# flawyer/Celebrity-Image-Denoiser

Hardware: AMD Instinct MI355X
Metric: images/sec at batch 256, 128x128x3, fp32 denoise forward (higher is better)
Workload: dtype f32

## Files before the change

celebrity_image_denoiser_amd/_lib.py:

```python
from __future__ import annotations

import ctypes
import os

_HERE = os.path.dirname(os.path.abspath(__file__))
LIB_PATH = os.environ.get("CID_LIB_PATH") or os.path.join(_HERE, "libcid.so")

CID_OK = 0
CID_NUM_PARAMS = 24
CID_NUM_LAUNCHES = 12
CID_ALGO_DIRECT, CID_ALGO_WINOGRAD64, CID_ALGO_WINOGRAD42, CID_ALGO_SPLIT16 = 0, 2, 3, 4
CID_FMT_F32_NCHW, CID_FMT_U8_NHWC = 0, 1
CID_DTYPE_F32, CID_DTYPE_F16 = 0, 1
CID_TAIL_FUSED, CID_TAIL_BANDS, CID_TAIL_TILES = 0, 1, 2
CID_METRIC_PSNR, CID_METRIC_SSIM, CID_METRIC_MS_SSIM = 1, 2, 4
CID_DISC_MOMENTUM_NONE = -1.0
CID_NOISE_GAUSSIAN, CID_NOISE_SALT_PEPPER, CID_NOISE_SPECKLE, CID_NOISE_POISSON, CID_NOISE_UNIFORM = 0, 1, 2, 3, 4
CID_ADAM_MAX_TENSORS = 32
CID_RESAMPLE_BICUBIC = 3
CID_SR_RAW = 1
CID_CG_RAW = 1
CID_LPIPS_UNIT_VIEW = 1
CID_LPIPS_NUM_WEIGHTS = 17

# ... 17 lines not shown
    "cid_set_weight": (_c.c_int, [_c.c_void_p, _c.c_char_p, _c.c_void_p, _c.POINTER(_c.c_int64), _c.c_int]),
    "cid_get_weight": (_c.c_int, [_c.c_void_p, _c.c_char_p, _c.c_void_p, _c.c_size_t]),
    "cid_missing_weights": (_c.c_int, [_c.c_void_p, _c.POINTER(_c.c_int)]),
    "cid_param_key": (_c.c_char_p, [_c.c_int]),
    "cid_packed_weights_bytes": (_c.c_size_t, []),
    "cid_upload_weights": (_c.c_int, [_c.c_void_p, _c.c_void_p, _c.c_void_p]),
    "cid_pack_weights_device": (_c.c_int, [_c.c_void_p, _c.c_void_p, _c.c_void_p, _c.c_void_p]),
    "cid_packed_segment": (_c.c_int, [_c.c_int, _c.POINTER(_c.c_char_p), _c.POINTER(_c.c_size_t), _c.POINTER(_c.c_size_t)]),
    "cid_export_packed": (_c.c_int, [_c.c_void_p, _c.c_void_p, _c.c_size_t]),
    "cid_import_packed": (_c.c_int, [_c.c_void_p, _c.c_void_p, _c.c_size_t]),
    "cid_attach_weights": (_c.c_int, [_c.c_void_p, _c.c_void_p]),
    "cid_out_shape": (_c.c_int, [_c.c_int, _c.c_int, _c.POINTER(_c.c_int), _c.POINTER(_c.c_int)]),
    "cid_workspace_bytes": (_c.c_int, [_c.c_int, _c.c_int, _c.c_int, _c.POINTER(_c.c_size_t)]),
    "cid_forward": (_c.c_int, [_c.c_void_p, _c.c_void_p, _c.c_void_p, _c.c_int, _c.c_int, _c.c_int,
                               _c.c_void_p, _c.c_size_t, _c.c_void_p]),
    "cid_forward_ex": (_c.c_int, [_c.c_void_p, _c.c_void_p, _c.c_int, _c.c_void_p, _c.c_int, _c.c_int, _c.c_int, _c.c_int,
                                  _c.c_void_p, _c.c_size_t, _c.c_void_p]),
    "cid_forward_padded": (_c.c_int, [_c.c_void_p, _c.c_void_p, _c.c_int, _c.c_void_p, _c.c_int, _c.c_int, _c.c_int, _c.c_int,
                                      _c.c_int, _c.c_int, _c.c_int, _c.c_int, _c.c_void_p, _c.c_size_t, _c.c_void_p]),
    "cid_view_u8": (_c.c_int, [_c.c_void_p, _c.c_void_p, _c.c_int, _c.c_int, _c.c_int, _c.c_void_p]),
    "cid_forward_timed": (_c.c_int, [_c.c_void_p, _c.c_void_p, _c.c_void_p, _c.c_int, _c.c_int, _c.c_int,
                                     _c.c_void_p, _c.c_size_t, _c.c_void_p, _c.POINTER(_c.c_float)]),
    "cid_timing_begin": (_c.c_int, [_c.c_void_p, _c.c_int]),
    "cid_timing_end": (_c.c_int, [_c.c_void_p, _c.c_void_p, _c.POINTER(_c.c_float), _c.POINTER(_c.c_int)]),
    "cid_launch_name": (_c.c_char_p, [_c.c_int]),
    "cid_launch_kernel": (_c.c_char_p, [_c.c_void_p, _c.c_int]),
    "cid_set_conv_algo": (_c.c_int, [_c.c_void_p, _c.c_int]),
    "cid_get_conv_algo": (_c.c_int, [_c.c_void_p, _c.POINTER(_c.c_int)]),
    "cid_set_tail_algo": (_c.c_int, [_c.c_void_p, _c.c_int]),
    "cid_get_tail_algo": (_c.c_int, [_c.c_void_p, _c.POINTER(_c.c_int)]),
    "cid_debug_poison_lds": (_c.c_int, [_c.c_void_p]),
    "cid_debug_winograd_workgroups_per_cu": (_c.c_int, [_c.c_int]),
    "cid_debug_half_workgroups_per_cu": (_c.c_int, [_c.c_int]),
    "cid_debug_winograd_column_block_per_xcd": (_c.c_int, [_c.c_int]),
    "cid_set_compute_dtype": (_c.c_int, [_c.c_void_p, _c.c_int]),
    "cid_get_compute_dtype": (_c.c_int, [_c.c_void_p, _c.POINTER(_c.c_int)]),
    "cid_launch_work_ex": (_c.c_int, [_c.c_void_p, _c.c_int, _c.c_int, _c.c_int, _c.c_int, _c.POINTER(_c.c_double), _c.POINTER(_c.c_double)]),
    "cid_stage_view": (_c.c_int, [_c.c_char_p, _c.c_int, _c.c_int, _c.c_int, _c.POINTER(_c.c_size_t), _c.POINTER(_c.c_int),
                                  _c.POINTER(_c.c_int), _c.POINTER(_c.c_int), _c.POINTER(_c.c_int), _c.POINTER(_c.c_int)]),
    "cid_comm_available": (_c.c_int, []),
    "cid_comm_unique_id": (_c.c_int, [_c.c_void_p]),
    "cid_comm_init_rank": (_c.c_int, [_c.POINTER(_c.c_void_p), _c.c_int, _c.c_void_p, _c.c_int]),
    "cid_comm_destroy": (_c.c_int, [_c.c_void_p]),
    "cid_comm_count": (_c.c_int, [_c.c_void_p, _c.POINTER(_c.c_int)]),
    "cid_broadcast_weights": (_c.c_int, [_c.c_void_p, _c.c_void_p, _c.c_int, _c.c_int, _c.c_void_p]),
    "cid_launch_work": (_c.c_int, [_c.c_int, _c.c_int, _c.c_int, _c.c_int, _c.POINTER(_c.c_double), _c.POINTER(_c.c_double)]),
    "cid_quality_workspace_bytes": (_c.c_int, [_c.c_int, _c.c_int, _c.c_int, _c.c_int, _c.POINTER(_c.c_size_t)]),
    "cid_quality": (_c.c_int, [_c.c_void_p, _c.c_int, _c.c_void_p, _c.c_int, _c.c_int, _c.c_int, _c.c_int, _c.c_int,
                               _c.c_void_p, _c.c_void_p, _c.c_size_t, _c.c_void_p]),
    "cid_add_noise": (_c.c_int, [_c.c_void_p, _c.c_void_p, _c.c_int, _c.c_int, _c.c_int, _c.c_int, _c.POINTER(_c.c_double), _c.c_int,
                                 _c.c_uint64, _c.c_uint64, _c.c_void_p]),
    "cid_disc_create": (_c.c_int, [_c.POINTER(_c.c_void_p)]),
    "cid_disc_destroy": (None, [_c.c_void_p]),
    "cid_disc_last_error": (_c.c_char_p, [_c.c_void_p]),
    "cid_disc_set_weight": (_c.c_int, [_c.c_void_p, _c.c_char_p, _c.c_void_p, _c.POINTER(_c.c_int64), _c.c_int]),
    "cid_disc_packed_weights_bytes": (_c.c_size_t, []),
    "cid_disc_upload_weights": (_c.c_int, [_c.c_void_p, _c.c_void_p, _c.c_void_p]),
    "cid_disc_workspace_bytes": (_c.c_int, [_c.c_int, _c.c_int, _c.c_int, _c.c_int, _c.POINTER(_c.c_size_t)]),
    "cid_disc_forward": (_c.c_int, [_c.c_void_p, _c.c_void_p, _c.c_int, _c.c_void_p, _c.c_int, _c.c_int, _c.c_int, _c.c_void_p,
                                    _c.c_int, _c.c_void_p, _c.c_size_t, _c.c_void_p]),
    "cid_disc_saved_bytes": (_c.c_int, [_c.c_int, _c.c_int, _c.c_int, _c.c_int, _c.POINTER(_c.c_size_t)]),
    "cid_disc_forward_saved": (_c.c_int, [_c.c_void_p, _c.c_void_p, _c.c_int, _c.c_void_p, _c.c_int, _c.c_int, _c.c_int, _c.c_void_p,
                                          _c.c_int, _c.c_void_p, _c.c_size_t, _c.c_void_p]),
    "cid_disc_backward_workspace_bytes": (_c.c_int, [_c.c_int, _c.c_int, _c.c_int, _c.c_int, _c.POINTER(_c.c_size_t)]),
    "cid_disc_backward": (_c.c_int, [_c.c_void_p, _c.c_void_p, _c.c_int, _c.c_void_p, _c.c_int, _c.c_int, _c.c_int, _c.c_void_p,
                                     _c.c_int, _c.c_void_p, _c.c_size_t, _c.c_void_p, _c.c_void_p, _c.c_size_t, _c.c_void_p]),
# ... 141 lines not shown
```

celebrity_image_denoiser_amd/csrc/cid_api.hip:

```cpp
#include "../../include/cid.h"
#include "conv_kernels.h"
#include "wino64_kernels.h"
#include "wino42_kernels.h"
#include "conv_kernels_f16.h"
#include "quality_kernels.h"
#include "noise_kernels.h"
#include "disc_kernels.h"
#include "disc_bwd_kernels.h"
#include "gen_bwd_kernels.h"
#include "gen_pack_kernels.h"
#include "optim_kernels.h"
#include "resize_kernels.h"
#include "esrgan_kernels.h"
#include "srgan_kernels.h"
#include "cgan_kernels.h"
#include "lpips_kernels.h"

#include <dlfcn.h>

#include <algorithm>
#include <atomic>
#include <cmath>

#include <cstdio>
// ... 187 lines not shown

enum Buf { T0, CAT1, P1, T1, CAT2, P2, T2, BT, T3, D2, T4, NBUF };
struct Plan { size_t off[NBUF]; size_t total_bytes; };
Plan make_plan(const Dims& d) {
    const size_t s0 = (size_t)d.N * d.H * d.W, s1 = (size_t)d.N * d.H1 * d.W1, s2 = (size_t)d.N * d.H2 * d.W2;
    const size_t su2 = (size_t)d.N * d.Hu2 * d.Wu2, su1 = (size_t)d.N * d.Hu1 * d.Wu1;
    const size_t sz[NBUF] = {s0 * 64, su1 * 128, s1 * 64, s1 * 128, su2 * 256, s2 * 128, s2 * 256, s2 * 256, su2 * 128, su2 * 128, su1 * 64};
    Plan p; size_t o = 0;
    for (int b = 0; b < NBUF; ++b) { p.off[b] = o; o = align_up(o + sz[b], 64); }
    p.total_bytes = o * sizeof(float);
    return p;
}

}

struct cid_handle_s {
    std::vector<float> staging;
    bool have[NL][2];
    const float* dev_blob = nullptr;
    std::string err;
    int dtype = CID_DTYPE_F32;
    int tail_algo = CID_TAIL_FUSED;
    int algo = CID_ALGO_WINOGRAD42;
    std::vector<hipEvent_t> tev;
    int tev_forwards = 0, tev_used = 0;
    cid_handle_s() : staging(kBlob.total, 0.f) {
        std::memset(have, 0, sizeof(have));
        stage_segments(staging.data(), kTables, nullptr);
    }
};

namespace {

struct Config { int dtype, algo, tail; };
Config config_of(cid_handle_t h) {
    return h ? Config{h->dtype, h->algo, h->tail_algo} : Config{CID_DTYPE_F32, CID_ALGO_DIRECT, CID_TAIL_BANDS};
}

enum class Kern {
    HEAD, HEAD_H16,
    GEMM,
    CONVT_S32,
    WINO64, WINO42,
    SPLIT, SPLIT_PAIR,
    H16, CONVT_T16,
    Z_WINO64, Z_WINO42, Z_SPLIT, Z_H16,
    TAIL_BANDS, TAIL_TILES, TAIL_H,
    TAIL_Z, TAIL_ZH,
};

Kern select_kernel(const Config& c, int i) {
    const LayerDef& L = kLayers[i];
    const bool f16 = c.dtype == CID_DTYPE_F16;
    const bool fused = c.tail == CID_TAIL_FUSED && (f16 || c.algo != CID_ALGO_DIRECT);
    switch (L.kind) {
        case HEAD: return f16 ? Kern::HEAD_H16 : Kern::HEAD;
        case TAIL:
            if (fused) return f16 ? Kern::TAIL_ZH : Kern::TAIL_Z;
            return f16 ? Kern::TAIL_H : c.tail == CID_TAIL_BANDS ? Kern::TAIL_BANDS : Kern::TAIL_TILES;
        case CONVT:
            if (f16) return Kern::CONVT_T16;
            if (c.algo == CID_ALGO_SPLIT16) return Kern::SPLIT_PAIR;
            return L.cin == 128 ? Kern::CONVT_S32 : Kern::GEMM;
        case CONV: break;
    }
    const bool z = fused && i == 10;
    if (f16) return z ? Kern::Z_H16 : Kern::H16;
    switch (c.algo) {
        case CID_ALGO_WINOGRAD64: return z ? Kern::Z_WINO64 : Kern::WINO64;
        case CID_ALGO_WINOGRAD42: return z ? Kern::Z_WINO42 : Kern::WINO42;
        case CID_ALGO_SPLIT16: return z ? Kern::Z_SPLIT : L.cout >= 128 ? Kern::SPLIT_PAIR : Kern::SPLIT;
        default: return Kern::GEMM;
    }
}

std::string kernel_name(const Config& c, int i) {
    const LayerDef& L = kLayers[i];
    const std::string dims = std::to_string(L.cin) + ", " + std::to_string(L.cout);
    const std::string mode = dims + ", " + std::to_string(mode_of(L)) + ",", pool = dims + (L.pool ? ", true," : ", false,");
    switch (select_kernel(c, i)) {
        case Kern::HEAD: return "k_conv_head";
        case Kern::HEAD_H16: return "k_conv_head_h16";
        case Kern::GEMM: return "k_gemm_conv<" + dims + ", " + std::to_string(mode_of(L));
        case Kern::CONVT_S32: return "k_convt_s32<" + dims + ">";
        case Kern::WINO64: case Kern::Z_WINO64: return "k_wino64_conv<" + pool;
        case Kern::WINO42: case Kern::Z_WINO42: return "k_wino42_conv<" + pool;
        case Kern::SPLIT: case Kern::SPLIT_PAIR: return "k_conv3x3_h16<" + mode + " false, false, true,";
        case Kern::H16: return "k_conv3x3_h16<" + mode + (i == 10 ? " false," : "");
        case Kern::CONVT_T16: return "k_convt_t16<" + dims + ">";
        case Kern::Z_SPLIT: return "k_conv3x3_h16<" + mode + " true, false, true,";
        case Kern::Z_H16: return "k_conv3x3_h16<" + mode + " true,";
        case Kern::TAIL_BANDS: case Kern::TAIL_TILES: return "k_conv_tail";
        case Kern::TAIL_H: return "k_conv_tail_h<";
        case Kern::TAIL_Z: return c.algo == CID_ALGO_SPLIT16 ? "k_conv_tail_z<" : "k_conv_tail";
        case Kern::TAIL_ZH: return "k_conv_tail_zh<";
    }
    return "";
}
struct KernelNames {
    std::string s[2][CID_ALGO_SPLIT16 + 1][3][NL];
    KernelNames() {
        for (int dt = 0; dt < 2; ++dt)
            for (int algo = 0; algo <= CID_ALGO_SPLIT16; ++algo)
                for (int tail = 0; tail < 3; ++tail)
                    for (int i = 0; i < NL; ++i) s[dt][algo][tail][i] = kernel_name(Config{dt, algo, tail}, i);
    }
};
const KernelNames kKernelNames;

int fail(cid_handle_t h, int code, const std::string& msg) {
    if (h) h->err = msg;
    return code;
}

bool find_key(const char* key, int& layer, int& is_bias) {
    if (!key) return false;
    const std::string k(key);
    for (int l = 0; l < NL; ++l) {
        const std::string n(kLayers[l].name);
        if (k == n + ".weight") { layer = l; is_bias = 0; return true; }
        if (k == n + ".bias") { layer = l; is_bias = 1; return true; }
    }
    return false;
}

inline int cdiv(int a, int b) { return (a + b - 1) / b; }

template <typename A>
void set_tiles(A& a, int N, int Hc, int Wc, int tw, int th) {
    a.tiles_x = cdiv(Wc, tw); a.tiles_y = cdiv(Hc, th); a.tiles_total = N * a.tiles_x * a.tiles_y;
    a.rcp_x = tile_rcp(a.tiles_x); a.rcp_xy = tile_rcp(a.tiles_x * a.tiles_y);
    if constexpr (std::is_same_v<A, HeadArgs> || std::is_same_v<A, TailArgs>) tile_groups(a);
    else a.tiles_per_xcd = cdiv(a.tiles_total, 8);
}

struct LayerIO {
    const float* in; int Hin, Win, in_ps;
    float* out; int out_ps, out_coff;
// ... 27 lines not shown
    if (hipGetDevice(&dev) != hipSuccess || dev < 0 || dev >= MAXDEV) return 256;
    int n = cache[dev].load(std::memory_order_relaxed);
    if (n > 0) return n;
    if (hipDeviceGetAttribute(&n, hipDeviceAttributeMultiprocessorCount, dev) != hipSuccess || n < 1) n = 256;
    cache[dev].store(n, std::memory_order_relaxed);
    return n;
}
int wino42_grid(WinoArgs& a, int nb) {
    const int per_cu = g_wino42_wg_per_cu;
    const int cus = device_cus();
    const int items = 8 * a.tiles_per_xcd * nb;
    const int walkers = per_cu * cus / 8;
    a.walk = 0;
    if (per_cu <= 0 || walkers < 1 || items <= 8 * walkers || a.tiles_per_xcd < walkers) return items;
    a.walk = walkers;
    if ((nb == 2 || nb == 4) && (g_wino42_xnb & nb)) {
        a.tiles_per_xcd = cdiv(a.tiles_total, 8 / nb);
        a.walk = -walkers;
    }
    return 8 * walkers;
}

template <int CIN, int COUT, int MODE>
hipError_t launch_gemm(const Ctx& x, int layer, const LayerIO& io) {
    GemmConvArgs a;
    set_layer_io(a, x.N, io);
    a.w = x.blob + kBlob.w_off[layer]; a.bias = x.blob + kBlob.b_off[layer];
    set_tiles(a, x.N, io.Hc, io.Wc, TILE_W, TILE_H);
    constexpr int NB = (MODE == 2 ? 4 * COUT : COUT) / NTILE;
    hipLaunchKernelGGL((k_gemm_conv<CIN, COUT, MODE>), dim3(8 * a.tiles_per_xcd * NB), dim3(THREADS), 0, x.s, a);
    return hipGetLastError();
}

template <int CIN, int COUT>
hipError_t launch_convt_s32(const Ctx& x, int layer, const LayerIO& io) {
    using CG = ConvTGeom32<CIN, COUT>;
    GemmConvArgs a;
    set_layer_io(a, x.N, io);
    a.w = x.blob + kBlob.w_off[layer]; a.bias = x.blob + kBlob.b_off[layer];
    a.tiles_x = (io.Hin * io.Win + CG::TP - 1) / CG::TP; a.tiles_y = 1; a.tiles_total = x.N * a.tiles_x; a.tiles_per_xcd = 0;
    a.rcp_x = tile_rcp(a.tiles_x); a.rcp_xy = tile_rcp(io.Win);
    const int wgs = device_cus() * 2;
    hipLaunchKernelGGL((k_convt_s32<CIN, COUT>), dim3(a.tiles_total < wgs ? a.tiles_total : wgs), dim3(THREADS), 0, x.s, a);
    return hipGetLastError();
}

template <bool ZOUT>
WinoArgs wino_args(const Ctx& x, int layer, const LayerIO& io, size_t u_off) {
    WinoArgs a;
    set_layer_io(a, x.N, io);
    a.u = x.blob + u_off; a.bias = x.blob + kBlob.b_off[layer];
    a.zw = ZOUT ? x.blob + kBlob.w_off[11] : nullptr; a.zout = ZOUT ? io.out : nullptr;
    if (ZOUT) a.out = nullptr;
    a.walk = 0;
    return a;
}

template <int CIN, int COUT, bool POOL, bool ZOUT>
hipError_t launch_wino64(const Ctx& x, int layer, const LayerIO& io) {
    WinoArgs a = wino_args<ZOUT>(x, layer, io, kBlob.u_off[layer]);
    const bool wide = io.Wc > 32;
    a.slot_tab = reinterpret_cast<const unsigned*>(x.blob + kBlob.tab_off[wide ? 0 : 1]);
    set_tiles(a, x.N, io.Hc, io.Wc, wide ? 64 : 32, wide ? 2 : 4);
    const dim3 grid(8 * a.tiles_per_xcd * (COUT / WN2));
    if (wide) hipLaunchKernelGGL((k_wino64_conv<CIN, COUT, POOL, 32, ZOUT>), grid, dim3(THREADS), 0, x.s, a);
    else hipLaunchKernelGGL((k_wino64_conv<CIN, COUT, POOL, 16, ZOUT>), grid, dim3(THREADS), 0, x.s, a);
    return hipGetLastError();
}

template <int CIN, int COUT, bool POOL, bool ZOUT>
hipError_t launch_wino42(const Ctx& x, int layer, const LayerIO& io) {
    WinoArgs a = wino_args<ZOUT>(x, layer, io, kBlob.u42_off[layer]);
    const bool wide = io.Wc > 16;
    a.slot_tab = reinterpret_cast<const unsigned*>(x.blob + kBlob.tab42_off[wide ? 0 : 1]);
    set_tiles(a, x.N, io.Hc, io.Wc, wide ? 32 : 16, wide ? 4 : 8);
    const dim3 grid(wino42_grid(a, COUT / WN2));
// ... 18 lines not shown

template <int CIN, int COUT, int MODE, bool ZOUT>
hipError_t launch_gemm_h(const Ctx& x, int layer, const LayerIO& io) {
    GemmConvArgsH a;
    set_layer_io(a, x.N, io);
    a.w = reinterpret_cast<const _Float16*>(x.blob + kBlob.h_off[layer]); a.bias = x.blob + kBlob.b_off[layer];
    if (ZOUT) a.pool = const_cast<_Float16*>(reinterpret_cast<const _Float16*>(x.blob + kBlob.hz_off));
    set_tiles(a, x.N, io.Hc, io.Wc, TILE_W, TILE_H);
    constexpr int NB = (MODE == 2 ? 4 * COUT : COUT) / NTILE;
    a.walk = 0;
    if constexpr (MODE == 2 && !ZOUT) {
        using CG = ConvTGeom<CIN, COUT>;
        a.tiles_x = (io.Hin * io.Win + CG::TP - 1) / CG::TP; a.tiles_total = x.N * a.tiles_x;
        a.rcp_x = tile_rcp(a.tiles_x); a.rcp_xy = tile_rcp(io.Win);
        const int wgs = device_cus() * 2 / CG::CB;
        hipLaunchKernelGGL((k_convt_t16<CIN, COUT>), dim3(a.tiles_total < wgs ? a.tiles_total : wgs), dim3(64 * CG::NW), 0, x.s, a);
    } else if constexpr (MODE != 2) {
        if (io.in_ps != CIN) return hipErrorInvalidValue;
        int grid = 8 * a.tiles_per_xcd * NB;
        const int walkers = g_half_wg_per_cu * device_cus() / 8;
        if (CIN <= 128 && g_half_wg_per_cu > 0 && walkers >= 1 && grid > 8 * walkers && a.tiles_per_xcd >= walkers) { a.walk = walkers; grid = 8 * walkers; }
        if constexpr (MODE == 0) {
            if (a.walk) { hipLaunchKernelGGL((k_conv3x3_h16<CIN, COUT, MODE, ZOUT, true>), dim3(grid), dim3(THREADS), 0, x.s, a); return hipGetLastError(); }
        }
        a.walk = 0; grid = 8 * a.tiles_per_xcd * NB;
        hipLaunchKernelGGL((k_conv3x3_h16<CIN, COUT, MODE, ZOUT, false>), dim3(grid), dim3(THREADS), 0, x.s, a);
    }
    return hipGetLastError();
}

template <int LAYER>
hipError_t launch_layer(const Ctx& x, const LayerIO& io) {
    constexpr int CIN = kLayers[LAYER].cin, COUT = kLayers[LAYER].cout, MODE = mode_of(kLayers[LAYER]);
    constexpr bool CONV = MODE != 2, Z = LAYER == 10, S32 = MODE == 2 && CIN == 128;
    switch (select_kernel(x.c, LAYER)) {
        case Kern::GEMM: if constexpr (!S32) return launch_gemm<CIN, COUT, MODE>(x, LAYER, io); break;
        case Kern::CONVT_S32: if constexpr (S32) return launch_convt_s32<CIN, COUT>(x, LAYER, io); break;
        case Kern::WINO64: if constexpr (CONV) return launch_wino64<CIN, COUT, MODE == 1, false>(x, LAYER, io); break;
        case Kern::WINO42: if constexpr (CONV) return launch_wino42<CIN, COUT, MODE == 1, false>(x, LAYER, io); break;
        case Kern::SPLIT: if constexpr (CONV && COUT < 128) return launch_split16<CIN, COUT, MODE, false, false>(x, LAYER, io); break;
        case Kern::SPLIT_PAIR: if constexpr (!CONV || COUT >= 128) return launch_split16<CIN, COUT, MODE, false, true>(x, LAYER, io); break;
        case Kern::H16: if constexpr (CONV) return launch_gemm_h<CIN, COUT, MODE, false>(x, LAYER, io); break;
        case Kern::CONVT_T16: if constexpr (!CONV) return launch_gemm_h<CIN, COUT, MODE, false>(x, LAYER, io); break;
        case Kern::Z_WINO64: if constexpr (Z) return launch_wino64<CIN, COUT, false, true>(x, LAYER, io); break;
        case Kern::Z_WINO42: if constexpr (Z) return launch_wino42<CIN, COUT, false, true>(x, LAYER, io); break;
        case Kern::Z_SPLIT: if constexpr (Z) return launch_split16<CIN, COUT, MODE, true, false>(x, LAYER, io); break;
        case Kern::Z_H16: if constexpr (Z) return launch_gemm_h<CIN, COUT, MODE, true>(x, LAYER, io); break;
        default: break;
    }
    return hipErrorInvalidValue;
}

hipError_t launch_head(const Ctx& x, const void* in, bool u8, const Window& src, float* out, int H, int W) {
    const bool f16 = select_kernel(x.c, 0) == Kern::HEAD_H16;
    HeadArgs a;
    a.in = in; a.w = x.blob + (f16 ? kBlob.h_off[0] : kBlob.w_off[0]); a.bias = x.blob + kBlob.b_off[0]; a.out = out;
    a.N = x.N; a.H = H; a.W = W; a.src = src;
    set_tiles(a, x.N, H, W, TILE_W, TILE_H);
    const dim3 grid(8 * a.groups_per_xcd);
    if (u8 && f16) hipLaunchKernelGGL((k_conv_head_h16<true>), grid, dim3(THREADS), 0, x.s, a);
    else if (u8) hipLaunchKernelGGL((k_conv_head<true>), grid, dim3(THREADS), 0, x.s, a);
    else if (f16) hipLaunchKernelGGL((k_conv_head_h16<false>), grid, dim3(THREADS), 0, x.s, a);
    else hipLaunchKernelGGL((k_conv_head<false>), grid, dim3(THREADS), 0, x.s, a);
    return hipGetLastError();
}

hipError_t launch_tail(const Ctx& x, const float* t4, void* out, bool u8, const Window& crop, int H, int W) {
    const Kern k = select_kernel(x.c, 11);
    const float* bias = x.blob + kBlob.b_off[11];
    if (k == Kern::TAIL_Z || k == Kern::TAIL_ZH) {
// ... 260 lines not shown
    const long long Hp = (long long)H + pad_top + pad_bottom, Wp = (long long)W + pad_left + pad_right;
    if (Hp > 0x7fffffff || Wp > 0x7fffffff) return fail(h, CID_ERR_SHAPE, "cid_forward_padded: padded size overflows");
    int Ho = 0, Wo = 0;
    if (cid_out_shape((int)Hp, (int)Wp, &Ho, &Wo) != CID_OK) return fail(h, CID_ERR_SHAPE, "cid_forward_padded: padded image smaller than 4x4 (output size is too small)");
    if (pad_top + H > Ho || pad_left + W > Wo) {
        char m[256];
        std::snprintf(m, sizeof m, "cid_forward_padded: the crop window [%d+%d, %d+%d] does not fit the network output %dx%d of the padded image %lldx%lld "
                                   "(pad to a multiple of 4, app.py:276-281)", pad_top, H, pad_left, W, Ho, Wo, Hp, Wp);
        return fail(h, CID_ERR_SHAPE, m);
    }
    const Window src{pad_top, pad_left, H, W}, crop{pad_top, pad_left, H, W};
    return run_forward(h, in, in_fmt, out, out_fmt, N, (int)Hp, (int)Wp, ws, ws_bytes, static_cast<hipStream_t>(stream), nullptr, &src, &crop);
}

int cid_view_u8(const float* in_nchw, void* out_u8_nhwc, int N, int H, int W, void* stream) {
    if (!in_nchw || !out_u8_nhwc || N < 1 || H < 1 || W < 1) return CID_ERR_INVALID;
    const size_t plane = (size_t)H * W, pixels = plane * N;
    if ((pixels + THREADS - 1) / THREADS > 0x7fffffffull) return CID_ERR_SHAPE;
    hipLaunchKernelGGL(k_view_u8, dim3((unsigned)((pixels + THREADS - 1) / THREADS)), dim3(THREADS), 0, static_cast<hipStream_t>(stream),
                       in_nchw, static_cast<unsigned char*>(out_u8_nhwc), plane, pixels);
    return hipGetLastError() == hipSuccess ? CID_OK : CID_ERR_HIP;
}

int cid_debug_winograd_workgroups_per_cu(int k) {
    const int prev = g_wino42_wg_per_cu;
    if (k >= 0) g_wino42_wg_per_cu = k > 2 ? 2 : k;
    return prev;
}
int cid_debug_winograd_column_block_per_xcd(int mask) {
    const int prev = g_wino42_xnb;
    if (mask >= 0) g_wino42_xnb = mask & 6;
    return prev;
}
int cid_debug_half_workgroups_per_cu(int k) {
    const int prev = g_half_wg_per_cu;
    if (k >= 0) g_half_wg_per_cu = k > 3 ? 3 : k;
    return prev;
}

int cid_timing_begin(cid_handle_t h, int max_forwards) {
    if (!h) return CID_ERR_INVALID;
    if (max_forwards < 1 || max_forwards > 4096) return fail(h, CID_ERR_INVALID, "cid_timing_begin: max_forwards out of range");
    if (!h->tev.empty()) return fail(h, CID_ERR_STATE, "cid_timing_begin: timing already armed");
    h->tev.resize((size_t)max_forwards * (NL + 1));
    for (size_t i = 0; i < h->tev.size(); ++i)
        if (hipEventCreate(&h->tev[i]) != hipSuccess) {
            for (size_t j = 0; j < i; ++j) (void)hipEventDestroy(h->tev[j]);
            h->tev.clear();
            return fail(h, CID_ERR_HIP, "cid_timing_begin: hipEventCreate failed");
        }
    h->tev_forwards = max_forwards;
    h->tev_used = 0;
    return CID_OK;
}

int cid_timing_end(cid_handle_t h, void* stream, float* launch_ms_sum, int* forwards) {
    if (!h) return CID_ERR_INVALID;
    if (!launch_ms_sum || !forwards) return fail(h, CID_ERR_INVALID, "cid_timing_end: null pointer");
    if (h->tev.empty()) return fail(h, CID_ERR_STATE, "cid_timing_end: timing not armed");
    int rc = CID_OK;
    if (hipStreamSynchronize(static_cast<hipStream_t>(stream)) != hipSuccess) rc = fail(h, CID_ERR_HIP, "cid_timing_end: stream sync failed");
    for (int l = 0; l < NL; ++l) launch_ms_sum[l] = 0.f;
    for (int f = 0; rc == CID_OK && f < h->tev_used; ++f)
        for (int l = 0; l < NL; ++l) {
            float ms = 0.f;
            const hipEvent_t* e = h->tev.data() + (size_t)f * (NL + 1);
            if (hipEventElapsedTime(&ms, e[l], e[l + 1]) != hipSuccess) { rc = fail(h, CID_ERR_HIP, "cid_timing_end: hipEventElapsedTime failed"); break; }
            launch_ms_sum[l] += ms;
        }
    *forwards = h->tev_used;
    for (hipEvent_t e : h->tev) (void)hipEventDestroy(e);
    h->tev.clear();
    h->tev_forwards = h->tev_used = 0;
    return rc;
}

int cid_forward_timed(cid_handle_t h, const float* in, float* out, int N, int H, int W, void* ws, size_t ws_bytes,
                      void* stream, float* launch_ms) {
    if (!h) return CID_ERR_INVALID;
    if (!launch_ms) return fail(h, CID_ERR_INVALID, "cid_forward_timed: null launch_ms");
    hipEvent_t ev[NL + 1];
    int made = 0;
    for (; made <= NL; ++made)
        if (hipEventCreate(&ev[made]) != hipSuccess) break;
    int rc = made == NL + 1 ? CID_OK : fail(h, CID_ERR_HIP, "hipEventCreate failed");
    hipStream_t s = static_cast<hipStream_t>(stream);
    if (rc == CID_OK) rc = run_forward(h, in, CID_FMT_F32_NCHW, out, CID_FMT_F32_NCHW, N, H, W, ws, ws_bytes, s, ev);
    if (rc == CID_OK && hipStreamSynchronize(s) != hipSuccess) rc = fail(h, CID_ERR_HIP, "cid_forward_timed: stream sync failed");
    if (rc == CID_OK)
        for (int l = 0; l < NL; ++l)
            if (hipEventElapsedTime(&launch_ms[l], ev[l], ev[l + 1]) != hipSuccess) rc = fail(h, CID_ERR_HIP, "hipEventElapsedTime failed");
    for (int i = 0; i < made; ++i) (void)hipEventDestroy(ev[i]);
    return rc;
}

const char* cid_launch_name(int i) { return (i >= 0 && i < NL) ? kLayers[i].name : nullptr; }
const char* cid_launch_kernel(cid_handle_t h, int i) {
    if (i < 0 || i >= NL) return nullptr;
    const Config c = config_of(h);
    return kKernelNames.s[c.dtype][c.algo][c.tail][i].c_str();
}

int cid_set_conv_algo(cid_handle_t h, int algo) {
    if (!h) return CID_ERR_INVALID;
    if (algo != CID_ALGO_DIRECT && algo != CID_ALGO_WINOGRAD64 && algo != CID_ALGO_WINOGRAD42 && algo != CID_ALGO_SPLIT16) return fail(h, CID_ERR_INVALID, "cid_set_conv_algo: unknown algorithm");
    h->algo = algo;
    return CID_OK;
}
int cid_set_tail_algo(cid_handle_t h, int algo) {
    if (!h) return CID_ERR_INVALID;
    if (algo != CID_TAIL_FUSED && algo != CID_TAIL_BANDS && algo != CID_TAIL_TILES) return fail(h, CID_ERR_INVALID, "cid_set_tail_algo: unknown algorithm");
    h->tail_algo = algo;
    return CID_OK;
}
int cid_get_tail_algo(cid_handle_t h, int* algo) {
    if (!h || !algo) return CID_ERR_INVALID;
    *algo = h->tail_algo;
    return CID_OK;
}
int cid_set_compute_dtype(cid_handle_t h, int dtype) {
    if (!h) return CID_ERR_INVALID;
    if (dtype != CID_DTYPE_F32 && dtype != CID_DTYPE_F16) return fail(h, CID_ERR_INVALID, "cid_set_compute_dtype: unknown dtype");
    h->dtype = dtype;
    return CID_OK;
}
int cid_get_compute_dtype(cid_handle_t h, int* dtype) {
    if (!h || !dtype) return CID_ERR_INVALID;
    *dtype = h->dtype;
    return CID_OK;
}
__global__ void __launch_bounds__(256) k_poison_lds() {
    __shared__ float lds[8192];
    for (int i = threadIdx.x; i < 8192; i += 256) lds[i] = __builtin_nanf("");
// ... 2882 lines not shown
```

celebrity_image_denoiser_amd/csrc/conv_kernels.h:

```cpp
#pragma once
#include <hip/hip_runtime.h>

#include <type_traits>

namespace cid {

typedef float f32x16 __attribute__((ext_vector_type(16)));
typedef float f32x4 __attribute__((ext_vector_type(4)));
typedef _Float16 f16x8 __attribute__((ext_vector_type(8)));
typedef _Float16 f16x4 __attribute__((ext_vector_type(4)));

constexpr int TILE_H = 8;
constexpr int TILE_W = 32;
constexpr int KCHUNK = 32;
constexpr int NTILE = 64;
constexpr int THREADS = 256;

struct GemmConvArgs {
    const float* in;
    const float* w;
    const float* bias;
    float* out;
    float* pool;
    int N, Hin, Win, in_ps;
// ... 931 lines not shown
                                acc[t][mt] = __builtin_amdgcn_mfma_f32_16x16x4f32(wf[g][j][mt], px[t][j], acc[t][mt], 0, 0, 0);
                            }
                        }
                __builtin_amdgcn_sched_barrier(0);
                if (g + 1 < G) {
#pragma unroll
                    for (int t = 0; t < TG; ++t) px[t] = pxn[t];
                }
            }
            if (has_next && t0 + TG == TN) asm volatile("s_waitcnt vmcnt(0)" ::: "memory");
#pragma unroll
            for (int t = 0; t < TG; ++t) {
                const unsigned q = (unsigned)(chunk * TP + (t0 + t) * 16 + c16);
                unsigned y = __umulhi(q, a.rcp_xy);
                int x = (int)(q - y * (unsigned)a.Win);
                if (a.Win == 1) { y = q; x = 0; }
                if (x < 0) { --y; x += a.Win; }
                const bool ok = (int)q < HW && (int)y < a.Hc && x < a.Wc;
                const unsigned po = ((2 * y + kh) * (unsigned)Wo + 2 * x + kw) * (unsigned)a.out_ps * 4 + lane_chan;
#pragma unroll
                for (int mt = 0; mt < 4; ++mt) {
                    const f32x4 v = acc[t][mt] + bias4[mt];
                    __builtin_amdgcn_raw_buffer_store_b128(__builtin_bit_cast(u32x4, v), ro, ok ? po + mt * 64 : 0x7ffffff0u, 0, 0);
                }
            }
        }
        if (!has_next) break;
        __syncthreads();
        tile = next;
        buf ^= 1;
    }
}

}
```

include/cid.h:

```cpp
#ifndef CID_H_
#define CID_H_

#include <stddef.h>
#include <stdint.h>

#ifdef __cplusplus
extern "C" {
#endif

typedef struct cid_handle_s* cid_handle_t;

enum {
    CID_OK = 0,
    CID_ERR_INVALID = 1,
    CID_ERR_SHAPE = 2,
    CID_ERR_KEY = 3,
    CID_ERR_STATE = 4,
    CID_ERR_WORKSPACE = 5,
    CID_ERR_HIP = 6
};

#define CID_NUM_PARAMS 24
#define CID_NUM_PARAM_ELEMS 1827587

// ... 189 lines not shown
int cid_cg_set_bn_eps(cid_cg_t h, int which, double eps);
int cid_cg_missing_weights(cid_cg_t h, int* count);
size_t cid_cg_packed_weights_bytes(cid_cg_t h);
int cid_cg_upload_weights(cid_cg_t h, void* device_blob, void* stream);
int cid_cg_workspace_bytes(int N, size_t* bytes);
int cid_cg_latent(uint64_t seed, uint64_t first_index, int N, float* z_out, void* stream);
int cid_cg_forward(cid_cg_t h, const float* z, const int64_t* labels, void* out, int out_fmt, int N, unsigned flags, void* workspace,
                   size_t workspace_bytes, void* stream);
int cid_cg_stage_view(const char* stage, int N, size_t* offset_bytes, int* C, int* Hs, int* Ws, int* channel_block);

typedef struct cid_lpips_s* cid_lpips_t;
enum { CID_LPIPS_UNIT_VIEW = 1 };
#define CID_LPIPS_NUM_WEIGHTS 17
int cid_lpips_create(cid_lpips_t* out);
void cid_lpips_destroy(cid_lpips_t h);
const char* cid_lpips_last_error(cid_lpips_t h);
const char* cid_lpips_param_key(cid_lpips_t h, int i);
int cid_lpips_set_weight(cid_lpips_t h, const char* key, const void* host_data, const int64_t* shape, int ndim);
int cid_lpips_missing_weights(cid_lpips_t h, int* count);
size_t cid_lpips_packed_weights_bytes(cid_lpips_t h);
int cid_lpips_upload_weights(cid_lpips_t h, void* device_blob, void* stream);
int cid_lpips_workspace_bytes(int N, int H, int W, size_t* bytes);
int cid_lpips_stage_view(const char* stage, int N, int H, int W, size_t* offset_bytes, int* C, int* Hs, int* Ws, int* channel_block);
int cid_lpips(cid_lpips_t h, const void* a, int fmt_a, const void* b, int fmt_b, int N, int H, int W, unsigned flags, double* out,
              double* layers, void* workspace, size_t workspace_bytes, void* stream);

int cid_debug_poison_lds(void* stream);
int cid_debug_adam_step_host(const cid_adam_tensor* tensors, int ntensors, const cid_adam_hyper* hp);
int cid_disc_saved_masks(const void* saved, size_t saved_bytes, int N, int H, int W, int training, unsigned char* const* masks,
                         void* stream);
int cid_debug_winograd_workgroups_per_cu(int k);
int cid_debug_winograd_column_block_per_xcd(int mask);
int cid_debug_half_workgroups_per_cu(int k);

#ifdef __cplusplus
}
#endif
#endif
```

profiles/summarize.py:

```python
#!/usr/bin/env python3
import csv
import glob
import json
import os
import shutil
import sys
from collections import defaultdict


EXPECT = ["k_conv_head<", "k_wino42_conv<64, 64, true,", "k_wino42_conv<64, 128, false,", "k_wino42_conv<128, 128, true,",
          "k_wino42_conv<128, 256, false,", "k_wino42_conv<256, 256, false,", "k_gemm_conv<256, 128, 2",
          "k_wino42_conv<256, 128, false,", "k_wino42_conv<128, 128, false,", "k_convt_s32<128, 64>",
          "k_wino42_conv<128, 64, false,", "k_conv_tail_z<"]


def one(pattern, what):
    found = sorted(glob.glob(pattern, recursive=True))
    if len(found) != 1:
        sys.exit(f"summarize.py: expected exactly one {what}, found {len(found)}: {found} — re-run profiles/collect.sh (it starts from an empty directory)")
    return found[0]


def short(name):
    name = name.replace("void cid::", "").replace("cid::", "")
    return name.split("(")[0]


def load_counters(d):
    vals, dur = defaultdict(lambda: defaultdict(list)), defaultdict(list)
    for f in [one(os.path.join(d, "**", "*_counter_collection.csv"), f"counter CSV under {d}")]:
        seen = set()
        for r in csv.DictReader(open(f)):
            k = short(r["Kernel_Name"])
            vals[k][r["Counter_Name"]].append(float(r["Counter_Value"]))
            if r["Dispatch_Id"] not in seen:
                seen.add(r["Dispatch_Id"])
                dur[k].append(float(r["End_Timestamp"]) - float(r["Start_Timestamp"]))
    mean = lambda v: sum(v) / len(v)
    return {k: {c: mean(v) for c, v in cs.items()} for k, cs in vals.items()}, {k: mean(v) for k, v in dur.items()}


def main():
    args = [a for a in sys.argv[1:] if not a.startswith("--")]
    allow_other = "--allow-other-kernels" in sys.argv
# ... 73 lines not shown
```

Measured before the change: 26680.

## Add persistent double-buffered MFMA kernel for 256->128 transposed conv

Adds k_convt_w32, a persistent transposed-convolution kernel for the 256-to-128 upsampling layer, and enables it by default in place of the generic GEMM conv. Each wave handles one of the four 2x2 taps. Input tiles are DMA'd into LDS with a swizzle and double-buffered so the next tile loads while the current one computes. Weights stream through a four-deep register ring ahead of the 32x32x2 f32 MFMA chain, and bias is added before direct buffer stores. The aim is to hide memory latency and make better use of MFMA on this layer, at the cost of high register pressure and a specialised code path.

New measurement: 26670, median of 2. No clear change (-0.0%).

```diff
diff --git a/celebrity_image_denoiser_amd/_lib.py b/celebrity_image_denoiser_amd/_lib.py
--- a/celebrity_image_denoiser_amd/_lib.py
+++ b/celebrity_image_denoiser_amd/_lib.py
@@ -73,6 +73,7 @@
     "cid_debug_poison_lds": (_c.c_int, [_c.c_void_p]),
     "cid_debug_winograd_workgroups_per_cu": (_c.c_int, [_c.c_int]),
     "cid_debug_half_workgroups_per_cu": (_c.c_int, [_c.c_int]),
+    "cid_debug_convt_walk": (_c.c_int, [_c.c_int]),
     "cid_debug_winograd_column_block_per_xcd": (_c.c_int, [_c.c_int]),
     "cid_set_compute_dtype": (_c.c_int, [_c.c_void_p, _c.c_int]),
     "cid_get_compute_dtype": (_c.c_int, [_c.c_void_p, _c.POINTER(_c.c_int)]),
diff --git a/celebrity_image_denoiser_amd/csrc/cid_api.hip b/celebrity_image_denoiser_amd/csrc/cid_api.hip
--- a/celebrity_image_denoiser_amd/csrc/cid_api.hip
+++ b/celebrity_image_denoiser_amd/csrc/cid_api.hip
@@ -243,7 +243,8 @@
 
 namespace {
 
-struct Config { int dtype, algo, tail; };
+int g_convt_walk = 1;
+struct Config { int dtype, algo, tail; int convt_walk = g_convt_walk; };
 Config config_of(cid_handle_t h) {
     return h ? Config{h->dtype, h->algo, h->tail_algo} : Config{CID_DTYPE_F32, CID_ALGO_DIRECT, CID_TAIL_BANDS};
 }
@@ -252,6 +253,7 @@
     HEAD, HEAD_H16,
     GEMM,
     CONVT_S32,
+    CONVT_W32,
     WINO64, WINO42,
     SPLIT, SPLIT_PAIR,
     H16, CONVT_T16,
@@ -272,7 +274,7 @@
         case CONVT:
             if (f16) return Kern::CONVT_T16;
             if (c.algo == CID_ALGO_SPLIT16) return Kern::SPLIT_PAIR;
-            return L.cin == 128 ? Kern::CONVT_S32 : Kern::GEMM;
+            return L.cin == 128 ? Kern::CONVT_S32 : c.convt_walk ? Kern::CONVT_W32 : Kern::GEMM;
         case CONV: break;
     }
     const bool z = fused && i == 10;
@@ -294,6 +296,7 @@
         case Kern::HEAD_H16: return "k_conv_head_h16";
         case Kern::GEMM: return "k_gemm_conv<" + dims + ", " + std::to_string(mode_of(L));
         case Kern::CONVT_S32: return "k_convt_s32<" + dims + ">";
+        case Kern::CONVT_W32: return "k_convt_w32<" + dims + ">";
         case Kern::WINO64: case Kern::Z_WINO64: return "k_wino64_conv<" + pool;
         case Kern::WINO42: case Kern::Z_WINO42: return "k_wino42_conv<" + pool;
         case Kern::SPLIT: case Kern::SPLIT_PAIR: return "k_conv3x3_h16<" + mode + " false, false, true,";
@@ -309,12 +312,13 @@
     return "";
 }
 struct KernelNames {
-    std::string s[2][CID_ALGO_SPLIT16 + 1][3][NL];
+    std::string s[2][CID_ALGO_SPLIT16 + 1][3][2][NL];
     KernelNames() {
         for (int dt = 0; dt < 2; ++dt)
             for (int algo = 0; algo <= CID_ALGO_SPLIT16; ++algo)
                 for (int tail = 0; tail < 3; ++tail)
-                    for (int i = 0; i < NL; ++i) s[dt][algo][tail][i] = kernel_name(Config{dt, algo, tail}, i);
+                    for (int walk = 0; walk < 2; ++walk)
+                        for (int i = 0; i < NL; ++i) s[dt][algo][tail][walk][i] = kernel_name(Config{dt, algo, tail, walk}, i);
     }
 };
 const KernelNames kKernelNames;
@@ -408,16 +412,15 @@
     return hipGetLastError();
 }
 
-template <int CIN, int COUT>
-hipError_t launch_convt_s32(const Ctx& x, int layer, const LayerIO& io) {
-    using CG = ConvTGeom32<CIN, COUT>;
+template <typename CG, void (*KERNEL)(const GemmConvArgs)>
+hipError_t launch_convt_walk(const Ctx& x, int layer, const LayerIO& io) {
     GemmConvArgs a;
     set_layer_io(a, x.N, io);
     a.w = x.blob + kBlob.w_off[layer]; a.bias = x.blob + kBlob.b_off[layer];
     a.tiles_x = (io.Hin * io.Win + CG::TP - 1) / CG::TP; a.tiles_y = 1; a.tiles_total = x.N * a.tiles_x; a.tiles_per_xcd = 0;
     a.rcp_x = tile_rcp(a.tiles_x); a.rcp_xy = tile_rcp(io.Win);
     const int wgs = device_cus() * 2;
-    hipLaunchKernelGGL((k_convt_s32<CIN, COUT>), dim3(a.tiles_total < wgs ? a.tiles_total : wgs), dim3(THREADS), 0, x.s, a);
+    hipLaunchKernelGGL(KERNEL, dim3(a.tiles_total < wgs ? a.tiles_total : wgs), dim3(THREADS), 0, x.s, a);
     return hipGetLastError();
 }
 
@@ -502,10 +505,11 @@
 template <int LAYER>
 hipError_t launch_layer(const Ctx& x, const LayerIO& io) {
     constexpr int CIN = kLayers[LAYER].cin, COUT = kLayers[LAYER].cout, MODE = mode_of(kLayers[LAYER]);
-    constexpr bool CONV = MODE != 2, Z = LAYER == 10, S32 = MODE == 2 && CIN == 128;
+    constexpr bool CONV = MODE != 2, Z = LAYER == 10, S32 = MODE == 2 && CIN == 128, W32 = MODE == 2 && CIN == 256;
     switch (select_kernel(x.c, LAYER)) {
         case Kern::GEMM: if constexpr (!S32) return launch_gemm<CIN, COUT, MODE>(x, LAYER, io); break;
-        case Kern::CONVT_S32: if constexpr (S32) return launch_convt_s32<CIN, COUT>(x, LAYER, io); break;
+        case Kern::CONVT_S32: if constexpr (S32) return launch_convt_walk<ConvTGeom32<CIN, COUT>, k_convt_s32<CIN, COUT>>(x, LAYER, io); break;
+        case Kern::CONVT_W32: if constexpr (W32) return launch_convt_walk<ConvTWalk32<CIN, COUT>, k_convt_w32<CIN, COUT>>(x, LAYER, io); break;
         case Kern::WINO64: if constexpr (CONV) return launch_wino64<CIN, COUT, MODE == 1, false>(x, LAYER, io); break;
         case Kern::WINO42: if constexpr (CONV) return launch_wino42<CIN, COUT, MODE == 1, false>(x, LAYER, io); break;
         case Kern::SPLIT: if constexpr (CONV && COUT < 128) return launch_split16<CIN, COUT, MODE, false, false>(x, LAYER, io); break;
@@ -832,6 +836,11 @@
     if (mask >= 0) g_wino42_xnb = mask & 6;
     return prev;
 }
+int cid_debug_convt_walk(int on) {
+    const int prev = g_convt_walk;
+    if (on >= 0) g_convt_walk = on ? 1 : 0;
+    return prev;
+}
 int cid_debug_half_workgroups_per_cu(int k) {
     const int prev = g_half_wg_per_cu;
     if (k >= 0) g_half_wg_per_cu = k > 3 ? 3 : k;
@@ -898,7 +907,7 @@
 const char* cid_launch_kernel(cid_handle_t h, int i) {
     if (i < 0 || i >= NL) return nullptr;
     const Config c = config_of(h);
-    return kKernelNames.s[c.dtype][c.algo][c.tail][i].c_str();
+    return kKernelNames.s[c.dtype][c.algo][c.tail][c.convt_walk ? 1 : 0][i].c_str();
 }
 
 int cid_set_conv_algo(cid_handle_t h, int algo) {
diff --git a/celebrity_image_denoiser_amd/csrc/conv_kernels.h b/celebrity_image_denoiser_amd/csrc/conv_kernels.h
--- a/celebrity_image_denoiser_amd/csrc/conv_kernels.h
+++ b/celebrity_image_denoiser_amd/csrc/conv_kernels.h
@@ -987,4 +987,166 @@
     }
 }
 
-}
+template <int CIN, int COUT>
+struct ConvTWalk32 {
+    static constexpr int NW = 4;
+    static constexpr int S = CIN / 4;
+    static constexpr int TP = 32;
+    static constexpr int PPR = NW * 64 / S;
+    static constexpr int ROUNDS = TP / PPR;
+    static constexpr int BUFQ = TP * S;
+    static constexpr int CB = COUT / NTILE;
+    static constexpr int KS = CIN / 8;
+    static_assert(CIN == 256 && COUT == 128, "up2");
+    static_assert(16 % PPR == 0 && S >= 16, "the swizzle term (p & 15) repeats every 16 / PPR rounds");
+};
+
+template <int CIN, int COUT>
+__global__ void __launch_bounds__(THREADS, 2) k_convt_w32(const GemmConvArgs a) {
+    using Gm = ConvTWalk32<CIN, COUT>;
+    constexpr int S = Gm::S, TP = Gm::TP, NW = Gm::NW, ROUNDS = Gm::ROUNDS, BUFQ = Gm::BUFQ, PPR = Gm::PPR, CB = Gm::CB, KS = Gm::KS;
+    constexpr int NV = 16 / PPR;
+    constexpr int NSTEP = CB * KS;
+    constexpr int NBUF = 4, DIST = NBUF - 1;
+    static_assert(NSTEP % NBUF == 0 && KS % 8 == 0, "the ring position of step 0 is the same in every run");
+    __shared__ f32x4 lds[2 * BUFQ];
+    const int tid = threadIdx.x, lane = tid & 63;
+    const int wave = __builtin_amdgcn_readfirstlane(tid >> 6);
+    const int tap = wave, kh = tap >> 1, kw = tap & 1;
+    const int i = lane & 31, h = lane >> 5;
+    int tile = blockIdx.x;
+    if (tile >= a.tiles_total) return;
+    const int HW = a.Hin * a.Win;
+
+    f32x4 bias4[CB][2][4];
+#pragma unroll
+    for (int cb = 0; cb < CB; ++cb)
+#pragma unroll
+        for (int ns = 0; ns < 2; ++ns)
+#pragma unroll
+            for (int q = 0; q < 4; ++q) bias4[cb][ns][q] = *reinterpret_cast<const f32x4*>(a.bias + cb * NTILE + ns * 32 + 8 * q + 4 * h);
+
+    const __amdgpu_buffer_rsrc_t rsrc_w = __builtin_amdgcn_make_buffer_rsrc((void*)a.w, (short)0, CIN * 4 * COUT * 4, 0x00020000);
+    const int wlane = tap * NSTEP * 2048 + lane * 16;
+    auto w_load = [&](int g, int ns) -> f32x4 {
+        return __builtin_bit_cast(f32x4, __builtin_amdgcn_raw_buffer_load_b128(rsrc_w, wlane, g * 2048 + ns * 1024, 0));
+    };
+
+    const int sp = lane & (S - 1);
+    int pl[NV];
+    unsigned dma_lane[NV];
+#pragma unroll
+    for (int v = 0; v < NV; ++v) {
+        pl[v] = ((v * NW + wave) * 64 + lane) / S;
+        dma_lane[v] = (unsigned)(pl[v] * a.in_ps * 4 + ((sp ^ (pl[v] & 15)) * 16));
+    }
+    auto image_rsrc = [&](int n) {
+        const unsigned long long p = (unsigned long long)(a.in + (size_t)n * HW * a.in_ps);
+        const unsigned lo = __builtin_amdgcn_readfirstlane((unsigned)p), hi = __builtin_amdgcn_readfirstlane((unsigned)(p >> 32));
+        return __builtin_amdgcn_make_buffer_rsrc((void*)(((unsigned long long)hi << 32) | lo), (short)0, HW * a.in_ps * 4, 0x00020000);
+    };
+    auto split = [&](int t, int& n, int& chunk) {
+        n = a.tiles_x > 1 ? (int)__umulhi((unsigned)t, a.rcp_x) : t;
+        chunk = t - n * a.tiles_x;
+        if (chunk < 0) { --n; chunk += a.tiles_x; }
+    };
+    auto dma_run = [&](int t, int buf, bool live) {
+        int n, chunk;
+        split(t, n, chunk);
+        const __amdgpu_buffer_rsrc_t rsrc = image_rsrc(n);
+#pragma unroll
+        for (int j = 0; j < ROUNDS; ++j) {
+            const int base = chunk * TP + (j / NV) * 16;
+            const int q = base + pl[j % NV];
+            const unsigned vo = (live && q < HW) ? dma_lane[j % NV] : 0x7ffffff0u;
+            __builtin_amdgcn_raw_ptr_buffer_load_lds(rsrc, (__attribute__((address_space(3))) void*)&lds[buf * BUFQ + (j * NW + wave) * 64], 16, vo,
+                                                     base * a.in_ps * 4, 0, 0);
+        }
+    };
+
+    int rd[8];
+#pragma unroll
+    for (int k = 0; k < 8; ++k) rd[k] = i * S + ((2 * k + h) ^ (i & 15));
+
+    const int Ho = 2 * a.Hc, Wo = 2 * a.Wc;
+    auto out_rsrc = [&](int n) {
+        const unsigned long long p = (unsigned long long)(a.out + (size_t)n * Ho * Wo * a.out_ps);
+        const unsigned lo = __builtin_amdgcn_readfirstlane((unsigned)p), hi = __builtin_amdgcn_readfirstlane((unsigned)(p >> 32));
+        return __builtin_amdgcn_make_buffer_rsrc((void*)(((unsigned long long)hi << 32) | lo), (short)0, Ho * Wo * a.out_ps * 4, 0x00020000);
+    };
+    const unsigned lane_chan = (unsigned)((a.out_coff + 4 * h) * 4);
+    typedef unsigned u32x4 __attribute__((ext_vector_type(4)));
+
+    f32x4 wq[NBUF][2];
+#pragma unroll
+    for (int d = 0; d < DIST; ++d) {
+        wq[d][0] = w_load(d, 0);
+        wq[d][1] = w_load(d, 1);
+    }
+    dma_run(tile, 0, true);
+    asm volatile("s_waitcnt vmcnt(0)" ::: "memory");
+    __syncthreads();
+    int buf = 0;
+    for (;;) {
+        const int next = tile + gridDim.x;
+        const bool has_next = next < a.tiles_total;
+        dma_run(has_next ? next : tile, buf ^ 1, has_next);
+
+        int n, chunk;
+        split(tile, n, chunk);
+        const __amdgpu_buffer_rsrc_t ro = out_rsrc(n);
+        unsigned vo;
+        {
+            const unsigned q = (unsigned)(chunk * TP + i);
+            unsigned y = __umulhi(q, a.rcp_xy);
+            int x = (int)(q - y * (unsigned)a.Win);
+            if (a.Win == 1) { y = q; x = 0; }
+            if (x < 0) { --y; x += a.Win; }
+            const bool ok = (int)q < HW && (int)y < a.Hc && x < a.Wc;
+            vo = ok ? ((2 * y + kh) * (unsigned)Wo + 2 * x + kw) * (unsigned)a.out_ps * 4 + lane_chan : 0x7ffffff0u;
+        }
+        const f32x4* tb = lds + buf * BUFQ;
+        f32x16 acc[2];
+        f32x4 px = tb[rd[0]], pxn;
+#pragma unroll
+        for (int g = 0; g < NSTEP; ++g) {
+            const int cb = g / KS, ks = g % KS;
+            if (g + 1 < NSTEP) {
+                const int k2 = (g + 1) % KS;
+                pxn = tb[rd[k2 & 7] + 16 * (k2 >> 3)];
+            }
+            wq[(g + DIST) % NBUF][0] = w_load((g + DIST) % NSTEP, 0);
+            wq[(g + DIST) % NBUF][1] = w_load((g + DIST) % NSTEP, 1);
+#pragma unroll
+            for (int e = 0; e < 4; ++e)
+#pragma unroll
+                for (int ns = 0; ns < 2; ++ns) {
+                    if (ks == 0 && e == 0) {
+                        const f32x16 zero = {0.f, 0.f, 0.f, 0.f, 0.f, 0.f, 0.f, 0.f, 0.f, 0.f, 0.f, 0.f, 0.f, 0.f, 0.f, 0.f};
+                        acc[ns] = __builtin_amdgcn_mfma_f32_32x32x2f32(wq[g % NBUF][ns][e], px[e], zero, 0, 0, 0);
+                    } else {
+                        acc[ns] = __builtin_amdgcn_mfma_f32_32x32x2f32(wq[g % NBUF][ns][e], px[e], acc[ns], 0, 0, 0);
+                    }
+                }
+            if (g + 1 < NSTEP) px = pxn;
+            __builtin_amdgcn_sched_barrier(0);
+            if (ks == KS - 1) {
+                if (cb == CB - 1) asm volatile("s_waitcnt vmcnt(%0)" ::"n"(2 * DIST) : "memory");
+#pragma unroll
+                for (int ns = 0; ns < 2; ++ns)
+#pragma unroll
+                    for (int q = 0; q < 4; ++q) {
+                        const f32x4 v = f32x4{acc[ns][4 * q], acc[ns][4 * q + 1], acc[ns][4 * q + 2], acc[ns][4 * q + 3]} + bias4[cb][ns][q];
+                        __builtin_amdgcn_raw_buffer_store_b128(__builtin_bit_cast(u32x4, v), ro, vo + (unsigned)((cb * NTILE + ns * 32 + 8 * q) * 4), 0, 0);
+                    }
+            }
+        }
+        if (!has_next) break;
+        __syncthreads();
+        tile = next;
+        buf ^= 1;
+    }
+    asm volatile("s_waitcnt vmcnt(0)" ::: "memory");
+}
+
+}
diff --git a/include/cid.h b/include/cid.h
--- a/include/cid.h
+++ b/include/cid.h
@@ -245,6 +245,7 @@
 int cid_debug_winograd_workgroups_per_cu(int k);
 int cid_debug_winograd_column_block_per_xcd(int mask);
 int cid_debug_half_workgroups_per_cu(int k);
+int cid_debug_convt_walk(int on);
 
 #ifdef __cplusplus
 }
diff --git a/profiles/summarize.py b/profiles/summarize.py
--- a/profiles/summarize.py
+++ b/profiles/summarize.py
@@ -9,7 +9,7 @@
 
 
 EXPECT = ["k_conv_head<", "k_wino42_conv<64, 64, true,", "k_wino42_conv<64, 128, false,", "k_wino42_conv<128, 128, true,",
-          "k_wino42_conv<128, 256, false,", "k_wino42_conv<256, 256, false,", "k_gemm_conv<256, 128, 2",
+          "k_wino42_conv<128, 256, false,", "k_wino42_conv<256, 256, false,", "k_convt_w32<256, 128>",
           "k_wino42_conv<256, 128, false,", "k_wino42_conv<128, 128, false,", "k_convt_s32<128, 64>",
           "k_wino42_conv<128, 64, false,", "k_conv_tail_z<"]
 
```
